# 0kam/alproj

Hardware: AMD Instinct MI355X
Metric: Gpoints/s projected (pinhole + Brown-Conrady, single pose) over the 100M-vertex DSM; CMA-ES iterations/s in `cma` (higher is better)
Workload: dtype f32

## Files before the change

### alproj_amd/csrc/alp_internal.h

```cpp
#pragma once

#include <hip/hip_runtime.h>

#include "host/alp_host.h"
#include "host/alp_buffer.h"

namespace alp {

#define ALP_HIP(expr)                                                                     \
    do {                                                                                  \
        hipError_t e__ = (expr);                                                          \
        if (e__ != hipSuccess)                                                            \
            return ::alp::fail(ALP_EHIP, "%s failed: %s (%s:%d)", #expr,                  \
                               hipGetErrorString(e__), __FILE__, __LINE__);               \
    } while (0)

struct DeviceMemory {
    static int alloc(void **p, size_t bytes) {
        const hipError_t e = hipMalloc(p, bytes);
        return e == hipSuccess ? ALP_OK : fail(ALP_EHIP, "hipMalloc of %zu bytes failed: %s", bytes, hipGetErrorString(e));
    }
    static void release(void *p) { hipFree(p); }
};
struct PinnedMemory {
    static int alloc(void **p, size_t bytes) {
        const hipError_t e = hipHostMalloc(p, bytes, hipHostMallocDefault);
        return e == hipSuccess ? ALP_OK : fail(ALP_EHIP, "hipHostMalloc of %zu bytes failed: %s", bytes, hipGetErrorString(e));
    }
    static void release(void *p) { hipHostFree(p); }
};
template <typename T = void> using DeviceBuffer = Buffer<DeviceMemory, T>;
template <typename T = void> using PinnedBuffer = Buffer<PinnedMemory, T>;

struct Event {
    Event() = default;
    Event(Event &&o) noexcept : e(o.e) { o.e = nullptr; }
    Event &operator=(Event &&o) noexcept {
        std::swap(e, o.e);
        return *this;
    }
    ~Event() {
        if (e) hipEventDestroy(e);
    }
    int ensure() {
        if (!e && hipEventCreate(&e) != hipSuccess) return fail(ALP_EHIP, "hipEventCreate failed");
        return ALP_OK;
    }
    operator hipEvent_t() const { return e; }
    hipEvent_t e = nullptr;
};

struct Context {
    bool ready = false;
    int device = -1;
    int cu_count = 0;
    hipStream_t stream = nullptr;
    hipEvent_t events[64] = {};
    void *scratch = nullptr;
    size_t scratch_cap = 0;
    void *comm = nullptr;
    int rank = 0;
    int world = 1;
};
Context &ctx();
int require_init();
int scratch_reserve(size_t bytes, void **out);

void ktime_begin();
void ktime_end();
struct KTimeScope {
    KTimeScope() { ktime_begin(); }
    ~KTimeScope() { ktime_end(); }
};


const char *raster_dev_flags();

void points_release_staging();

int comm_allreduce_sum_f64(double *dev_buf, int64_t count);

}
```

### alproj_amd/csrc/alp_points.hip

```cpp
#include "alp_internal.h"

#include <algorithm>
#include <cmath>
#include <cstdlib>
#include <vector>

#include "alp_point_kernels.h"
#include "alp_points_internal.h"


using namespace alp;

using alp::host::CONFIRM_MAX;

namespace {

int alloc_planes(DeviceBuffer<> &slab, int k, int64_t n_pad, size_t es, void **planes[]) {
    if (int rc = slab.reserve((size_t)k * n_pad * es)) return rc;
    ALP_HIP(hipMemsetAsync(slab, 0, (size_t)k * n_pad * es, ctx().stream));
    for (int i = 0; i < k; ++i) *planes[i] = (char *)slab + (size_t)i * n_pad * es;
    return ALP_OK;
}

template <typename TIn, typename T>
__global__ __launch_bounds__(256) void column_to_plane_kernel(const TIn *__restrict__ src, int64_t count, int64_t dst_off, double o,
                                                              T *__restrict__ plane) {
    const int64_t stride = (int64_t)gridDim.x * blockDim.x;
    for (int64_t i = (int64_t)blockIdx.x * blockDim.x + threadIdx.x; i < count; i += stride)
        plane[dst_off + i] = (T)((double)src[i] - o);
}

template <typename TIn, typename Launch>
int staged_upload(const void *const *srcs, int nsrc, int64_t n, int width, int64_t CH, Launch launch) {
    const int64_t ch = n < CH ? (n > 0 ? n : 1) : CH;
    DeviceBuffer<TIn> stage;
    if (int rc = stage.reserve((size_t)ch * width * sizeof(TIn))) return rc;
    int rc = ALP_OK;
    for (int c = 0; c < nsrc && !rc; ++c)
        for (int64_t off = 0; off < n; off += ch) {
            const int64_t cnt = (n - off < ch) ? (n - off) : ch;
            hipError_t e = hipMemcpyAsync(stage, (const TIn *)srcs[c] + off * width, (size_t)cnt * width * sizeof(TIn),
                                          hipMemcpyHostToDevice, ctx().stream);
            if (e != hipSuccess) { rc = fail(ALP_EHIP, "H2D upload: %s", hipGetErrorString(e)); break; }
            launch(c, stage, cnt, off, (int)((cnt + 255) / 256 < 4096 ? (cnt + 255) / 256 : 4096));
            e = hipGetLastError();
            if (e != hipSuccess) { rc = fail(ALP_EHIP, "upload kernel: %s", hipGetErrorString(e)); break; }
        }
    if (hipStreamSynchronize(ctx().stream) != hipSuccess && !rc) rc = fail(ALP_EHIP, "upload: stream failed");
    return rc;
}

template <typename TIn, typename T, int C>
int upload_t(const void *rows, const void *const *cols, int64_t n, const double *o, void *const *planes) {
    if (cols)
        return staged_upload<TIn>(cols, C, n, 1, (int64_t)48 << 20, [&](int c, const TIn *stage, int64_t cnt, int64_t off, int grid) {
            hipLaunchKernelGGL((column_to_plane_kernel<TIn, T>), dim3(grid), dim3(256), 0, ctx().stream, stage, cnt, off, o[c], (T *)planes[c]);
        });
    return staged_upload<TIn>(&rows, 1, n, C, (int64_t)16 << 20, [&](int, const TIn *stage, int64_t cnt, int64_t off, int grid) {
        hipLaunchKernelGGL((aos_to_planes_kernel<TIn, T, C>), dim3(grid), dim3(256), 0, ctx().stream, stage, cnt, off, o[0], o[1], o[2],
                           (T *)planes[0], (T *)planes[1], (T *)planes[2]);
    });
}

template <int C>
int upload(const void *rows, const void *const *cols, int in_dtype, int64_t n, const double *o, int precision, void *const *planes) {
    if (in_dtype == ALP_F64 && precision == ALP_F64) return upload_t<double, double, C>(rows, cols, n, o, planes);
    if (in_dtype == ALP_F64 && precision == ALP_F32) return upload_t<double, float, C>(rows, cols, n, o, planes);
    if (in_dtype == ALP_F32 && precision == ALP_F64) return upload_t<float, double, C>(rows, cols, n, o, planes);
    if (in_dtype == ALP_F32 && precision == ALP_F32) return upload_t<float, float, C>(rows, cols, n, o, planes);
    return fail(ALP_EINVAL, "in_dtype must be ALP_F32 or ALP_F64");
}

int stream_grid(int64_t items) { return host::stream_grid(items, ctx().cu_count); }

constexpr uint32_t GRID_MAX_ROW = 64 << 10;
constexpr uint32_t GRID_NONE = 0xffffffffu;

template <typename B>
__global__ __launch_bounds__(256) void grid_row_length_kernel(const B *__restrict__ y, uint32_t n, uint32_t *flags) {
    const B y0 = y[0];
    uint32_t first = GRID_NONE;
    const uint32_t stride = gridDim.x * blockDim.x;
    for (uint32_t i = blockIdx.x * blockDim.x + threadIdx.x; i < n; i += stride)
        if (y[i] != y0) {
            first = i;
            break;
        }
    for (int m = 32; m >= 1; m >>= 1) {
        const uint32_t o = (uint32_t)__shfl_xor((int)first, m);
        first = o < first ? o : first;
    }
    if ((threadIdx.x & 63) == 0 && first != GRID_NONE) atomicMin(flags, first);
}

template <typename B>
__global__ __launch_bounds__(256) void grid_verify_kernel(const B *__restrict__ x, const B *__restrict__ y, uint32_t n, RowDiv rd,
                                                          uint32_t *flags) {
    bool ok = true;
    const uint32_t stride = gridDim.x * blockDim.x;
    for (uint32_t i = blockIdx.x * blockDim.x + threadIdx.x; i < n; i += stride) {
        const uint32_t r = rd.div(i);
        ok &= (x[i] == x[i - r * rd.w]) & (y[i] == y[r * rd.w]);
    }
    if (!ok) atomicOr(flags + 1, 1u);
}

// ... 363 lines not shown
    return comm_allreduce_sum_f64(sums, (int64_t)K * (T + 1));
}

template <typename TS>
int normal_batch_impl(alp_points *p, const std::vector<JacPlan> &plans, int loss, double f_scale, double *out, const int32_t *row_of_pose) {
    const int64_t B = (int64_t)plans.size();
    const int D = plans[0].D, T = D * (D + 1) / 2 + D + 1;
    const host::NormalGrid g = host::normal_batch_grid(p->n, B, ctx().cu_count);
    const size_t plans_bytes = round_up((int64_t)(B * sizeof(JacPlan)), 256), rows_bytes = row_of_pose ? round_up(B * 4, 256) : 0;
    char *dev = nullptr;
    if (int rc = scratch_reserve(plans_bytes + rows_bytes + ((size_t)B * g.blocks * T + (size_t)B * (T + 1)) * sizeof(double), (void **)&dev)) return rc;
    JacPlan *plans_dev = (JacPlan *)dev;
    int *rows_dev = (int *)(dev + plans_bytes);
    double *partials = (double *)(dev + plans_bytes + rows_bytes), *sums = partials + (size_t)B * g.blocks * T;
    hipStream_t st = ctx().stream;
    NormalPosesLaunch l;
    l.timed = true;
    if (g.blocks > 0) {
        const char *order = getenv("ALP_NORMAL_BATCH_ORDER");
        if (order) l.pose_in_x = !strcmp(order, "pose");
        ALP_HIP(hipMemcpyAsync(plans_dev, plans.data(), (size_t)B * sizeof(JacPlan), hipMemcpyHostToDevice, st));
        if (row_of_pose) {
            ALP_HIP(hipMemcpyAsync(rows_dev, row_of_pose, (size_t)B * 4, hipMemcpyHostToDevice, st));
            l.table = true;
            l.row_of_pose = rows_dev;
        }
    }
    if (int rc = normal_poses_enqueue<TS>(p, plans_dev, (int)B, D, g, loss, f_scale, l, partials, sums)) return rc;
    ALP_HIP(hipMemcpyAsync(out, sums, (size_t)B * (T + 1) * sizeof(double), hipMemcpyDeviceToHost, st));
    ALP_HIP(hipStreamSynchronize(st));
    return ALP_OK;
}

}

namespace alp {
int normal_listed_launch(alp_points *p, const JacPlan *plans, const int *list, const long long *count, const int *running, int K, int D,
                         const host::NormalGrid &g, int loss, double f_scale, double *partials, double *sums, bool weight_rows) {
    NormalPosesLaunch l;
    l.list = list, l.count = count, l.running = running, l.pose_in_x = 1, l.table = weight_rows;
    return p->precision == ALP_F64 ? normal_poses_enqueue<double>(p, plans, K, D, g, loss, f_scale, l, partials, sums)
                                   : normal_poses_enqueue<float>(p, plans, K, D, g, loss, f_scale, l, partials, sums);
}
int popeval_launch(alp_points *p, int64_t P, int loss_kind, double f_scale, bool lens_free, bool shared_pose, bool batched,
                   const double *params_dev) {
    return p->precision == ALP_F64 ? popeval_launch_t<double>(p, P, loss_kind, f_scale, lens_free, shared_pose, batched, params_dev)
                                   : popeval_launch_t<float>(p, P, loss_kind, f_scale, lens_free, shared_pose, batched, params_dev);
}
int points_pop_reserve(alp_points *p, int64_t P) { return ensure_pop_scratch(p, P, 0); }
}

namespace {
constexpr int64_t FETCH_CHUNK = (int64_t)8 << 20;
void *g_fetch_stage[2] = {nullptr, nullptr};
hipEvent_t g_fetch_ev[2] = {nullptr, nullptr};

using alp::host::convert_threads;
using alp::host::fetch_threads;

template <typename S, typename D>
__global__ __launch_bounds__(256) void cast_plane_kernel(const S *__restrict__ src, D *__restrict__ dst, long long n) {
    const long long stride = (long long)gridDim.x * blockDim.x;
    for (long long i = (long long)blockIdx.x * blockDim.x + threadIdx.x; i < n; i += stride) dst[i] = (D)src[i];
}

template <typename S, typename D>
int fetch_converted_t(alp_points *p, D *u_out, D *v_out) {
    hipStream_t st = ctx().stream;
    const S *planes[2] = {(const S *)p->u, (const S *)p->v};
    D *outs[2] = {u_out, v_out};
    const char *mode = getenv("ALP_FETCH_CONVERT");
    const bool on_device = mode ? !strcmp(mode, "device") : sizeof(D) < sizeof(S);
    if (on_device) {
        D *tmp = nullptr;
        if (int rc = scratch_reserve((size_t)FETCH_CHUNK * sizeof(D), (void **)&tmp)) return rc;
        for (int pl = 0; pl < 2; ++pl)
            for (int64_t off = 0; off < p->n; off += FETCH_CHUNK) {
                const int64_t cnt = std::min(FETCH_CHUNK, p->n - off);
                hipLaunchKernelGGL((cast_plane_kernel<S, D>), dim3(stream_grid(cnt)), dim3(256), 0, st, planes[pl] + off, tmp, (long long)cnt);
                ALP_HIP(hipMemcpyAsync(outs[pl] + off, tmp, (size_t)cnt * sizeof(D), hipMemcpyDeviceToHost, st));
            }
        ALP_HIP(hipStreamSynchronize(st));
        return ALP_OK;
    }
    for (auto &b : g_fetch_stage)
        if (!b) ALP_HIP(hipHostMalloc(&b, (size_t)FETCH_CHUNK * 8, hipHostMallocDefault));
    const int T = fetch_threads();
    for (auto &e : g_fetch_ev)
        if (!e) ALP_HIP(hipEventCreateWithFlags(&e, hipEventDisableTiming));
    hipEvent_t *ev = g_fetch_ev;
    struct Job { int pl; int64_t off, cnt; };
    std::vector<Job> jobs;
    for (int pl = 0; pl < 2; ++pl)
        for (int64_t off = 0; off < p->n; off += FETCH_CHUNK) jobs.push_back({pl, off, std::min(FETCH_CHUNK, p->n - off)});
    for (size_t k = 0; k <= jobs.size(); ++k) {
        if (k < jobs.size()) {
            const Job &j = jobs[k];
            ALP_HIP(hipMemcpyAsync(g_fetch_stage[k & 1], planes[j.pl] + j.off, (size_t)j.cnt * sizeof(S), hipMemcpyDeviceToHost, st));
            ALP_HIP(hipEventRecord(ev[k & 1], st));
        }
        if (k > 0) {
            const Job &j = jobs[k - 1];
            ALP_HIP(hipEventSynchronize(ev[(k - 1) & 1]));
            convert_threads((const S *)g_fetch_stage[(k - 1) & 1], outs[j.pl] + j.off, j.cnt, T);
        }
    }
    return ALP_OK;
}

}
namespace alp {
void points_release_staging() {
    for (auto &b : g_fetch_stage) {
        if (b) hipHostFree(b);
        b = nullptr;
    }
    for (auto &e : g_fetch_ev) {
        if (e) hipEventDestroy(e);
        e = nullptr;
    }
}
}
namespace {
int fetch_converted(alp_points *p, void *u_out, void *v_out, int out_dtype) {
    return out_dtype == ALP_F64 ? fetch_converted_t<float, double>(p, (double *)u_out, (double *)v_out)
                                : fetch_converted_t<double, float>(p, (float *)u_out, (float *)v_out);
}
}

namespace {
template <typename TIn, typename T>
int weights_stored(const void *w, int64_t n, std::vector<T> &out, double *sum) {
    const TIn *src = (const TIn *)w;
    out.resize((size_t)n);
    double s = 0;
    for (int64_t i = 0; i < n; ++i) {
        const double v = (double)src[i];
        if (!(v >= 0.0) || !std::isfinite(v))
            return fail(ALP_EINVAL, "alp_points_set_weights: weight %lld is negative, NaN or infinite", (long long)i);
        const T t = (T)v;
        if (!std::isfinite((double)t)) return fail(ALP_EINVAL, "alp_points_set_weights: weight %lld does not fit the set's element type", (long long)i);
        out[(size_t)i] = t;
        s += (double)t;
    }
    *sum = s;
    return ALP_OK;
}

template <typename T>
int set_weights_t(alp_points *p, const void *w, int in_dtype) {
    std::vector<T> stored;
    double sum = 0;
    if (int rc = in_dtype == ALP_F64 ? weights_stored<double, T>(w, p->n, stored, &sum) : weights_stored<float, T>(w, p->n, stored, &sum)) return rc;
    if (!p->w) {
        DeviceBuffer<> plane;
        if (int rc = plane.reserve((size_t)p->n_pad * sizeof(T))) return rc;
        hipError_t e = hipMemsetAsync(plane, 0, (size_t)p->n_pad * sizeof(T), ctx().stream);
// ... 503 lines not shown
```

### alproj_amd/csrc/alp_raster.hip

```cpp
#include "alp_raster_internal.h"

#include <algorithm>
#include <atomic>
#include <climits>
#include <cmath>
#include <cstdlib>
#include <thread>
#include <type_traits>
#include <vector>

namespace alp {

#include "raster_dev.h"
#include "raster_common.h"
#include "raster_parked.h"
#include "raster_index.h"
#include "raster_plan.h"
#include "raster_grid.h"
#include "raster_large.h"
#include "raster_resolve.h"
#include "raster_post.h"

}

using namespace alp;

namespace alp {

int upload_chunked(void *dst, const void *src, size_t bytes) {
    const size_t CH = (size_t)256 << 20;
    for (size_t off = 0; off < bytes; off += CH) {
        const size_t n = bytes - off < CH ? bytes - off : CH;
        ALP_HIP(hipMemcpyAsync((char *)dst + off, (const char *)src + off, n, hipMemcpyHostToDevice, ctx().stream));
    }
    ALP_HIP(hipStreamSynchronize(ctx().stream));
    return ALP_OK;
}

template <typename Launch>
static hipError_t staged_upload(const void *src, size_t esize, int64_t total, int64_t chunk, void *stage, Launch launch) {
    for (int64_t off = 0; off < total; off += chunk) {
        const int64_t cnt = total - off < chunk ? total - off : chunk;
        hipError_t e = hipMemcpyAsync(stage, (const char *)src + (size_t)off * esize, (size_t)cnt * esize, hipMemcpyHostToDevice, ctx().stream);
        if (e != hipSuccess) return e;
        launch(off, cnt);
        if ((e = hipGetLastError()) != hipSuccess) return e;
    }
    return hipSuccess;
}

int ensure_queue(alp_mesh *m, unsigned cap) {
    if (m->queue && m->qcap >= cap) return ALP_OK;
    m->qcap = 0;
    if (int rc = m->queue.reserve((size_t)cap * sizeof(WorkItem))) return rc;
    m->qcap = cap;
    return ALP_OK;
}

unsigned initial_queue_cap() { return host::initial_queue_cap(getenv("ALP_QUEUE_CAP")); }
// ... 281 lines not shown
        ALP_HIP(hipMemsetAsync(m->vis, 0, (size_t)v.w * v.h * sizeof(unsigned long long) + QC_TOTAL * sizeof(unsigned), st));
    if (m->n_tri > 0 && !resolve_only) {
        if (m->implicit)
            if (int e = ensure_grid_plan(m, p)) return e;
        if (int e = m->implicit ? draw_grid_mesh(m, v, p) : draw_indexed_mesh(m, v, p)) return e;
    }
    if (int e = m->implicit ? resolve_frame<true>(m, v, rc, min_distance, p) : resolve_frame<false>(m, v, rc, min_distance, p)) return e;
    m->last_v = v;
    m->last_rc = rc;
    m->last_min_distance = min_distance;
    m->unchecked = m->n_tri > 0;
    m->vis_current = true;
    m->rz_n = -1;
    ++(resolve_only ? m->frames_resolve_only : m->frames_full);
    if (int e = dev_report_frame(st)) return e;
    m->rendered = true;
    return ALP_OK;
}

static bool same_view(const View &a, const View &b) {
    return a.w == b.w && a.h == b.h && a.fx == b.fx && a.fy == b.fy && a.sx == b.sx && a.sy == b.sy && a.fxd == b.fxd && a.fyd == b.fyd &&
           !memcmp(a.R, b.R, sizeof(a.R)) && !memcmp(a.camf, b.camf, sizeof(a.camf)) && !memcmp(a.caml, b.caml, sizeof(a.caml)) &&
           !memcmp(a.Rd, b.Rd, sizeof(a.Rd)) && !memcmp(a.camd, b.camd, sizeof(a.camd));
}

int finish_frame(alp_mesh *m) {
    while (m->unchecked) {
        ALP_HIP(hipStreamSynchronize(ctx().stream));
        m->unchecked = false;
        host::FrameQueues have;
        have.items = m->qcap;
        have.general = m->gcap;
        for (int k = 0; k < 3; ++k) {
            have.park[k] = m->park_cap[k];
            have.park_b[k] = m->park_cap_b[k];
        }
        const host::QueueVerdict want = host::frame_verdict(m->qcount_host, QC_STRIDE, m->park_small != nullptr, have);
        if (want.none()) break;
        if (want.park)
            if (int e = alloc_park(m, want.caps.park, want.caps.park_b)) return e;
        if (want.items)
            if (int e = ensure_queue(m, want.caps.items)) return e;
        if (want.general)
            if (int e = ensure_gqueue(m, want.caps.general)) return e;
        if (int e = render_impl(m, m->last_v, m->last_rc, m->last_min_distance)) return e;
    }
    return ALP_OK;
}

}

int alp::finish_frame_of(alp_mesh *m) { return finish_frame(m); }

int alp::upload_f32(float *dst, const void *src, int dtype, int64_t n_vert) {
    const size_t count = (size_t)n_vert * 3;
    if (dtype == ALP_F32) return upload_chunked(dst, src, count * 4);
    const size_t CH = (size_t)24 << 20;
    const size_t ch = count < CH ? count : CH;
    double *stage = nullptr;
    if (int rc = scratch_reserve(ch * 8, (void **)&stage)) return rc;
    hipStream_t st = ctx().stream;
    const hipError_t e = staged_upload(src, 8, (int64_t)count, (int64_t)ch, stage, [&](int64_t off, int64_t cnt) {
        hipLaunchKernelGGL(cast_f64_f32_kernel, dim3(4096), dim3(256), 0, st, stage, (long long)cnt, (long long)off, dst);
    });
    if (e != hipSuccess) return fail(ALP_EHIP, "float64 upload: %s", hipGetErrorString(e));
    ALP_HIP(hipStreamSynchronize(st));
    return ALP_OK;
}

static int streamed_grid_check(alp_mesh *m, const void *ind, int ind_dtype, int64_t n_tri, long long gw, bool *is_grid) {
    hipStream_t st = ctx().stream;
    const size_t esize = ind_dtype == ALP_I32 ? 4 : 8;
    const int64_t total = n_tri * 3;
    const int64_t CH = (int64_t)(((size_t)192 << 20) / esize) / 3 * 3;
    const int64_t ch = total < CH ? total : CH;
    void *stage = nullptr;
    if (int rc = scratch_reserve((size_t)ch * esize, &stage)) return rc;
    hipError_t e = hipMemsetAsync(m->qcount_dev, 0, sizeof(unsigned), st);
    if (e == hipSuccess)
        e = staged_upload(ind, esize, total, ch, stage, [&](int64_t off, int64_t cnt) {
            if (ind_dtype == ALP_I32)
                hipLaunchKernelGGL(check_grid_chunk_kernel<int>, dim3(4096), dim3(256), 0, st, (const int *)stage, cnt / 3, off / 3, gw, m->qcount_dev);
            else
                hipLaunchKernelGGL(check_grid_chunk_kernel<long long>, dim3(4096), dim3(256), 0, st, (const long long *)stage, cnt / 3, off / 3, gw,
                                   m->qcount_dev);
        });
    if (e == hipSuccess) e = hipMemcpyAsync(m->qcount_host, m->qcount_dev, sizeof(unsigned), hipMemcpyDeviceToHost, st);
    if (e == hipSuccess) e = hipStreamSynchronize(st);
    if (e != hipSuccess) return fail(ALP_EHIP, "grid check: %s", hipGetErrorString(e));
    *is_grid = *m->qcount_host == 0;
    return ALP_OK;
}

static int upload_indices(alp_mesh *m, const void *ind, int ind_dtype) {
    hipStream_t st = ctx().stream;
    const long long n_vert = m->n_vert;
    if (int rc = m->ind.reserve((size_t)m->n_tri * 12)) return rc;
    if (hipMemsetAsync(m->qcount_dev, 0, sizeof(unsigned), st) != hipSuccess) return fail(ALP_EHIP, "index check: memset");
    const int64_t total = m->n_tri * 3;
    hipError_t e = hipSuccess;
    if (ind_dtype == ALP_I32) {
        if (int rc = upload_chunked(m->ind, ind, (size_t)total * 4)) return rc;
        hipLaunchKernelGGL(check_index_range_kernel, dim3(4096), dim3(256), 0, st, m->ind, (long long)total, n_vert, m->qcount_dev);
    } else {
        const int64_t CH = 24 << 20;
        const int64_t ch = total < CH ? total : CH;
        long long *stage = nullptr;
        if (int rc = scratch_reserve((size_t)ch * 8, (void **)&stage)) return rc;
        e = staged_upload(ind, 8, total, ch, stage, [&](int64_t off, int64_t cnt) {
            hipLaunchKernelGGL(narrow_indices_kernel, dim3(4096), dim3(256), 0, st, stage, (long long)cnt, (long long)off, m->ind, n_vert,
                               m->qcount_dev);
        });
    }
    if (e == hipSuccess) e = hipGetLastError();
    if (e == hipSuccess) e = hipMemcpyAsync(m->qcount_host, m->qcount_dev, sizeof(unsigned), hipMemcpyDeviceToHost, st);
    if (e == hipSuccess) e = hipStreamSynchronize(st);
    if (e != hipSuccess) return fail(ALP_EHIP, "index upload: %s", hipGetErrorString(e));
    if (*m->qcount_host == 0) return ALP_OK;
    for (int64_t i = 0; i < total; ++i) {
        const long long v = ind_dtype == ALP_I32 ? (long long)((const int *)ind)[i] : ((const long long *)ind)[i];
        if (v < 0 || v >= n_vert) return fail(ALP_EINVAL, "index %lld out of range at %lld", v, (long long)i);
    }
    return fail(ALP_EINVAL, "%u indices out of range", *m->qcount_host);
}

using alp::host::HostGridCheck;
using alp::host::host_check_threads;

extern "C" {

int alp_mesh_create(const void *vert, int vert_dtype, const void *value, int value_dtype, int64_t n_vert, const void *ind,
                    int ind_dtype, int64_t n_tri, int64_t grid_h, int64_t grid_w, alp_mesh_t **out) {
    if (int rc = require_init()) return rc;
    ALP_REQUIRE(out, "out is NULL");
    *out = nullptr;
    ALP_REQUIRE(vert && n_vert > 0, "vert is NULL or empty");
    ALP_REQUIRE(vert_dtype == ALP_F32 || vert_dtype == ALP_F64, "vert_dtype must be ALP_F32 or ALP_F64");
    ALP_REQUIRE(!value || value_dtype == ALP_F32 || value_dtype == ALP_F64, "value_dtype must be ALP_F32 or ALP_F64");
    ALP_REQUIRE(n_vert < ((int64_t)1 << 31), "more than 2^31 vertices");
    const bool implicit = ind == nullptr;
    if (implicit) {
        ALP_REQUIRE(grid_h >= 2 && grid_w >= 2 && grid_h * grid_w == n_vert, "implicit grid: grid_h*grid_w != n_vert");
        n_tri = 2 * (grid_h - 1) * (grid_w - 1);
    } else {
        ALP_REQUIRE(ind_dtype == ALP_I32 || ind_dtype == ALP_I64, "ind_dtype must be ALP_I32 or ALP_I64");
        ALP_REQUIRE(n_tri >= 0, "n_tri is negative");
    }
    ALP_REQUIRE(n_tri < ((int64_t)1 << 32) - 1, "more than 2^32-2 triangles");
    alp_mesh *m = new alp_mesh();
    m->n_vert = n_vert;
    m->n_tri = n_tri;
    m->grid_h = grid_h;
// ... 385 lines not shown
```

### alproj_amd/csrc/host/alp_host.h

```cpp
#pragma once

#include <algorithm>
#include <atomic>
#include <cmath>
#include <cstdarg>
#include <cstdint>
#include <cstdio>
#include <cstdlib>
#include <cstring>
#include <thread>
#include <vector>

#include "alproj_hip.h"

#if defined(__SANITIZE_THREAD__)
#define ALP_TSAN_BUILD 1
#elif defined(__has_feature)
#if __has_feature(thread_sanitizer)
#define ALP_TSAN_BUILD 1
#endif
#endif
#ifndef ALP_TSAN_BUILD
#define ALP_TSAN_BUILD 0
#endif
// ... 42 lines not shown
int fold_pose_jacobian(const double params[ALP_NPARAM], const double origin[3], const int32_t *target, int D, double *jac);

struct alignas(16) JacPlan {
    double rec[POSE_WORDS];
    double drow[JAC_MAX][12];
    double lens_f[JAC_MAX];
    double su, sv;
    int32_t lens_w[JAC_MAX];
    int32_t D;
};
int jacobian_plan(const double params[ALP_NPARAM], const double origin[3], const int32_t *target, int D, int of_residuals,
                  JacPlan *plan);

}
#include "host/alp_jacplan.h"
#include "host/alp_lm.h"
namespace alp {

namespace host {

constexpr int64_t HASH_SLICE_BYTES = (int64_t)8 << 20;
constexpr int64_t MINMAX_VALUES_PER_THREAD = (int64_t)1 << 20;
uint64_t hash64(const void *buf, int64_t bytes, int threads);
void minmax(const double *values, int64_t n, int threads, double out[2]);
void prefault(void *buf, int64_t bytes, int threads);

template <typename S, typename D>
inline void convert_slice(const S *__restrict__ src, D *__restrict__ dst, int64_t n) {
#if defined(__has_builtin) && __has_builtin(__builtin_nontemporal_store) && !ALP_TSAN_BUILD
    for (int64_t i = 0; i < n; ++i) __builtin_nontemporal_store((D)src[i], dst + i);
#else
    for (int64_t i = 0; i < n; ++i) dst[i] = (D)src[i];
#endif
}

constexpr int64_t CONVERT_SERIAL_BELOW = 1 << 16;

template <typename S, typename D>
inline void convert_threads(const S *src, D *dst, int64_t n, int T) {
    if (T <= 1 || n < CONVERT_SERIAL_BELOW) return convert_slice(src, dst, n);
    std::vector<std::thread> th;
    const int64_t per = ((n + T - 1) / T + 15) & ~(int64_t)15;
    for (int t = 1; t < T; ++t) {
        const int64_t a = std::min(n, per * t), b = std::min(n, per * (t + 1));
        if (b > a) th.emplace_back([=] { convert_slice(src + a, dst + a, b - a); });
    }
    convert_slice(src, dst, std::min(n, per));
    for (auto &x : th) x.join();
}

inline int fetch_threads() {
    if (const char *e = getenv("ALP_HOST_THREADS")) return std::max(1, std::min(64, atoi(e)));
    return (int)std::max(1u, std::min(16u, std::thread::hardware_concurrency()));
}

template <typename I>
inline void grid_rows_check(const I *ind, long long gw, long long row0, long long row1, std::atomic<bool> *bad) {
    const long long gc = gw - 1;
    for (long long r = row0; r < row1 && !bad->load(std::memory_order_relaxed); ++r) {
        const I *p = ind + (size_t)r * gc * 6;
        long long a = r * gw;
        bool diff = false;
        for (long long c = 0; c < gc; ++c, ++a, p += 6)
            diff |= (long long)p[0] != a || (long long)p[1] != a + gw || (long long)p[2] != a + gw + 1 || (long long)p[3] != a ||
                    (long long)p[4] != a + gw + 1 || (long long)p[5] != a + 1;
        if (diff) bad->store(true, std::memory_order_relaxed);
    }
}

struct HostGridCheck {
    std::vector<std::thread> threads;
    std::atomic<bool> bad{false};
    bool started = false;
    void start(const void *ind, int ind_dtype, long long gh, long long gw, int n_threads) {
        const long long rows = gh - 1;
        const int T = (int)std::min<long long>(n_threads, rows);
        try {
            for (int t = 0; t < T; ++t) {
                const long long r0 = rows * t / T, r1 = rows * (t + 1) / T;
                if (ind_dtype == ALP_I32) threads.emplace_back(grid_rows_check<int>, (const int *)ind, gw, r0, r1, &bad);
                else threads.emplace_back(grid_rows_check<long long>, (const long long *)ind, gw, r0, r1, &bad);
            }
            started = true;
        } catch (...) {
            bad.store(true);
            join();
            bad.store(false);
            started = false;
        }
    }
    void join() {
        for (auto &t : threads)
            if (t.joinable()) t.join();
        threads.clear();
    }
    bool is_grid() {
        join();
        return started && !bad.load();
    }
    ~HostGridCheck() { bad.store(true); join(); }
};

inline int host_check_threads(int64_t n_tri) {
    if (const char *e = getenv("ALP_HOST_THREADS")) return std::max(0, std::min(64, atoi(e)));
    if (n_tri < (1 << 18)) return 0;
    const unsigned hc = std::thread::hardware_concurrency();
// ... 73 lines not shown
```

### alproj_amd/csrc/host/alp_host_selfcheck.cpp

```cpp
#include <cinttypes>
#include <mutex>
#include <random>
#include <string>
#include <utility>

#include "host/alp_host.h"
#include "host/alp_buffer.h"

using namespace alp;

namespace {

std::atomic<int> g_failures{0};
std::mutex g_print;

#define CHECK(cond, ...)                                           \
    do {                                                           \
        if (!(cond)) {                                             \
            std::lock_guard<std::mutex> lk(g_print);               \
            fprintf(stderr, "CHECK FAILED %s:%d: %s | ", __FILE__, __LINE__, #cond); \
            fprintf(stderr, __VA_ARGS__);                          \
            fprintf(stderr, "\n");                                 \
            g_failures.fetch_add(1);                               \
        }                                                          \
// ... 111 lines not shown
        for (int k = 0; k < 8; ++k) {
            const double q[3] = {2000 * U(rng), 2000 * U(rng), 300 * U(rng)};
            const double P[3] = {origin[0] + q[0] - p[0], origin[1] + q[1] - p[1], origin[2] + q[2] - p[2]};
            double cam[3];
            for (int i = 0; i < 3; ++i) cam[i] = R[i][0] * P[0] + R[i][1] * P[1] + R[i][2] * P[2];
            const double x = fx * cam[0] + p[23] * cam[2], y = fy * cam[1] + p[24] * cam[2], z = cam[2];
            const double x1 = ((w - x / z) - c0) / c0, y1 = (y / z - c1) / c1;
            const double zf = rec[8] * q[0] + rec[9] * q[1] + rec[10] * q[2] + rec[11];
            const double x1f = (rec[0] * q[0] + rec[1] * q[1] + rec[2] * q[2] + rec[3]) / zf;
            const double y1f = (rec[4] * q[0] + rec[5] * q[1] + rec[6] * q[2] + rec[7]) / zf;
            if (std::fabs(z) < 1) continue;
            CHECK(std::fabs(x1f - x1) <= 1e-9 * std::max(1.0, std::fabs(x1)), "x1 %.17g vs %.17g", x1f, x1);
            CHECK(std::fabs(y1f - y1) <= 1e-9 * std::max(1.0, std::fabs(y1)), "y1 %.17g vs %.17g", y1f, y1);
            double pl[ALP_NPARAM];
            memcpy(pl, p, sizeof(pl));
            for (int i = 9; i <= 20; ++i) pl[i] = 0;
            CHECK(pose_is_lens_free(pl) && !pose_is_lens_free(p), "pose_is_lens_free");
            double lf[POSE_WORDS];
            fold_pose_lens_free(pl, origin, lf);
            const double uo = 5616 * U(rng), vo = 3744 * U(rng);
            const double u_ref = c0 * x1 + c0, v_ref = c1 * (y1 * (1 + pl[7]) / (1 + pl[8])) + c1;
            const double zl = lf[8] * q[0] + lf[9] * q[1] + lf[10] * q[2] + lf[11];
            const double du = (uo - lf[26]) + (lf[0] * q[0] + lf[1] * q[1] + lf[2] * q[2] + lf[3]) / zl;
            const double dv = (vo - lf[27]) + (lf[4] * q[0] + lf[5] * q[1] + lf[6] * q[2] + lf[7]) / zl;
            CHECK(std::fabs(du - (uo - u_ref)) <= 1e-8 * std::max(1.0, std::fabs(u_ref)), "lens-free du %.17g vs %.17g", du, uo - u_ref);
            CHECK(std::fabs(dv - (vo - v_ref)) <= 1e-8 * std::max(1.0, std::fabs(v_ref)), "lens-free dv %.17g vs %.17g", dv, vo - v_ref);
            CHECK(zl == zf && lf[26] == c0 && lf[27] == c1 && lf[12] == 0 && lf[31] == 0, "lens-free record layout");
        }
    }
}

template <typename S, typename D>
void check_convert_t() {
    const int64_t lim = host::CONVERT_SERIAL_BELOW;
    const int64_t sizes[] = {0, 1, 15, 16, 17, lim - 1, lim, lim + 1, 70001, (1 << 20) + 3};
    std::mt19937_64 rng(4);
    std::uniform_real_distribution<double> U(-1e7, 1e7);
    for (int64_t n : sizes) {
        std::vector<S> src((size_t)n);
        for (auto &x : src) x = (S)U(rng);
        for (int T : THREAD_COUNTS) {
            std::vector<D> dst((size_t)n, (D)-1);
            host::convert_threads(src.data(), dst.data(), n, T);
            bool same = true;
            for (int64_t i = 0; i < n; ++i) same &= dst[(size_t)i] == (D)src[(size_t)i];
            CHECK(same, "convert n=%" PRId64 " T=%d", n, T);
        }
    }
}

void check_convert() {
    check_convert_t<float, double>();
    check_convert_t<double, float>();
}

template <typename I>
std::vector<I> grid_indices(long long gh, long long gw) {
    std::vector<I> ind;
    ind.reserve((size_t)((gh - 1) * (gw - 1) * 6));
    for (long long r = 0; r + 1 < gh; ++r)
        for (long long c = 0; c + 1 < gw; ++c) {
            const long long a = r * gw + c;
            for (long long v : {a, a + gw, a + gw + 1, a, a + gw + 1, a + 1}) ind.push_back((I)v);
        }
    return ind;
}

template <typename I>
void check_grid_t(int dtype) {
    const long long shapes[][2] = {{2, 2}, {3, 5}, {17, 4}, {2, 300}, {300, 251}};
    for (auto &sh : shapes) {
        const long long gh = sh[0], gw = sh[1];
        std::vector<I> ind = grid_indices<I>(gh, gw);
        const int64_t n_tri = (int64_t)ind.size() / 3, n_vert = gh * gw;
        long long cgh = 0, cgw = 0;
        CHECK(host::grid_candidate(ind.data(), dtype, n_tri, n_vert, &cgh, &cgw) && cgh == gh && cgw == gw, "candidate %lld x %lld", gh, gw);
        CHECK(!host::grid_candidate(ind.data(), dtype, n_tri - 1, n_vert, &cgh, &cgw), "odd triangle count accepted");
        CHECK(!host::grid_candidate(ind.data(), dtype, n_tri, n_vert + 1, &cgh, &cgw) || (n_vert + 1) % gw == 0, "wrong vertex count accepted");
        for (int T : {1, 2, 8, 64}) {
            {
                host::HostGridCheck chk;
                chk.start(ind.data(), dtype, gh, gw, T);
                CHECK(chk.is_grid(), "grid %lld x %lld not recognised (T=%d)", gh, gw, T);
            }
            for (size_t at : {(size_t)0, ind.size() / 2, ind.size() - 1}) {
                const I keep = ind[at];
                ind[at] = (I)(keep + 1);
                {
                    host::HostGridCheck chk;
                    chk.start(ind.data(), dtype, gh, gw, T);
                    CHECK(!chk.is_grid(), "wrong entry %zu of a %lld x %lld grid not seen (T=%d)", at, gh, gw, T);
                }
                ind[at] = keep;
            }
            {
                host::HostGridCheck chk;
                chk.start(ind.data(), dtype, gh, gw, T);
            }
            {
                host::HostGridCheck chk;
                CHECK(!chk.is_grid(), "a check that never ran says grid");
            }
        }
    }
}

// ... 657 lines not shown
    }
    {
        Bytes a;
        CHECK(a.reserve(16) == ALP_OK, "reserve");
        unsigned char *pa = a;
        Bytes b(std::move(a));
        CHECK(!a && a.capacity() == 0 && b.get() == pa && b.capacity() == 16 && Mem::live == 1, "move construction");
        Bytes c;
        c = std::move(b);
        CHECK(!b && c.get() == pa && c.capacity() == 16 && Mem::live == 1, "move assignment to an empty buffer");
        Bytes d;
        CHECK(d.reserve(32) == ALP_OK && Mem::live == 2, "reserve");
        d = std::move(c);
        CHECK(!c && d.get() == pa && d.capacity() == 16 && Mem::live == 1, "move assignment onto a block left %d live", Mem::live);
        Bytes &self = d;
        d = std::move(self);
        CHECK(d.get() == pa && Mem::live == 1, "self-assignment");
        Buffer<Mem> v;
        CHECK(v.reserve(8) == ALP_OK && (const float *)v == (const float *)v.get() && (char *)v + 4 == (char *)v.get() + 4, "casts");
    }
    CHECK(Mem::live == 0, "%d block(s) outlived their buffers", Mem::live);
    for (int size = 2; size <= 3; ++size)
        for (int bad = 1; bad <= size; ++bad)
            for (int held = 0; held < 2; ++held) {
                Buffer<Mem, double> x;
                Buffer<Mem> y;
                Buffer<Mem, int> z;
                auto group = [&](size_t n) {
                    return size == 2 ? reserve_all({n, 2 * n}, x, y) : reserve_all({n, 2 * n, 3 * n}, x, y, z);
                };
                if (held) CHECK(group(8) == ALP_OK && Mem::live == size, "first group");
                Mem::fail_next(bad);
                CHECK(group(64) == ALP_EHIP && !x && !y && !z && x.capacity() + y.capacity() + z.capacity() == 0 && Mem::live == 0,
                      "group of %d, member %d failed (held %d): %d block(s) live", size, bad, held, Mem::live);
                Mem::fail_next(0);
                CHECK(group(64) == ALP_OK && x && y && (size == 2 || z) && x.capacity() == 64 && y.capacity() == 128,
                      "group of %d after a failure", size);
                CHECK(Mem::live == size, "group of %d after a failure: %d blocks", size, Mem::live);
                x[7] = 1.0;
                ((char *)y)[127] = 1;
                if (size == 3) z[47] = 1;
                double *px = x;
                CHECK(group(64) == ALP_OK && x.get() == px && Mem::live == size, "a group that fits moved");
                reset_all(x, y, z);
                CHECK(Mem::live == 0, "reset_all");
            }
    CHECK(Mem::live == 0, "%d block(s) live at the end", Mem::live);
}

int main(int argc, char **argv) {
    if (argc > 2 && !strcmp(argv[1], "--canary")) return canary(argv[2]);
    if (argc > 1 && !strcmp(argv[1], "--plan")) return plan(argc - 2, argv + 2);
    if (argc > 1 && !strcmp(argv[1], "--lm")) return lm_mode();
    struct Group { const char *name; void (*fn)(); };
    const Group groups[] = {{"hash", check_hash},     {"minmax", check_minmax},   {"prefault", check_prefault}, {"fold_pose", check_fold_pose},
                            {"convert", check_convert}, {"grid", check_grid},     {"selection", check_selection}, {"errors", check_errors},
                            {"plan", check_plan},       {"frame_plan", check_frame_plan}, {"row_div", check_row_div}, {"lm", check_lm},
                            {"buffer", check_buffer},   {"row_walk", check_row_walk}, {"match_plan", check_match_plan}};
    const bool concurrent = !(argc > 1 && !strcmp(argv[1], "--serial"));
    std::vector<std::thread> th;
    for (const Group &g : groups) {
        if (concurrent) th.emplace_back(g.fn);
        else g.fn();
    }
    for (auto &x : th) x.join();
    std::thread a(check_convert), b(check_convert);
    check_selection();
    a.join();
    b.join();
    if (g_failures.load()) {
        fprintf(stderr, "host selfcheck: %d comparison(s) failed\n", g_failures.load());
        return 1;
    }
    printf("host selfcheck ok: %zu groups%s\n", sizeof(groups) / sizeof(groups[0]), concurrent ? ", run concurrently" : "");
    return 0;
}
```

Baseline: 502.1.

## Narrow float64 coordinates and int64 indices on host before upload

Adds a host-side multithreaded narrowing path that converts float64 vertex columns (optionally subtracting an origin) and int64 triangle indices to 32-bit values in pinned double-buffered staging. The narrowed data is copied to the device with async copies that overlap the next chunk's conversion. This halves the bytes crossing PCIe and drops the device-side conversion kernels. In exchange it uses host CPU threads and moves the index range check to the host. The staging buffers are now shared with the fetch path.

After: 499.8. Within noise of the previous version (-0.5%).

```diff
diff --git a/alproj_amd/csrc/alp_internal.h b/alproj_amd/csrc/alp_internal.h
--- a/alproj_amd/csrc/alp_internal.h
+++ b/alproj_amd/csrc/alp_internal.h
@@ -76,7 +76,43 @@
 
 const char *raster_dev_flags();
 
+constexpr size_t HOST_STAGE_BYTES = (size_t)64 << 20;
+int host_staging(void *stage[2], hipEvent_t ev[2]);
 void points_release_staging();
+
+inline bool narrow_on_host() {
+    const char *mode = getenv("ALP_UPLOAD_CONVERT");
+    return !mode || strcmp(mode, "device") != 0;
+}
+
+inline int64_t narrow_chunk_values() {
+    const int64_t most = (int64_t)(HOST_STAGE_BYTES / 4);
+    const char *e = getenv("ALP_UPLOAD_CHUNK");
+    return e ? std::max<int64_t>(1, std::min<int64_t>(most, atoll(e))) : most;
+}
+
+template <typename Narrow>
+inline int upload_narrowed(void *dst, int64_t total, Narrow narrow) {
+    void *stage[2];
+    hipEvent_t ev[2];
+    if (int rc = host_staging(stage, ev)) return rc;
+    hipStream_t st = ctx().stream;
+    const int64_t ch = narrow_chunk_values();
+    hipError_t e = hipSuccess;
+    int64_t k = 0;
+    for (int64_t off = 0; off < total && e == hipSuccess; off += ch, ++k) {
+        const int64_t cnt = std::min(ch, total - off);
+        const int b = (int)(k & 1);
+        if (k >= 2) e = hipEventSynchronize(ev[b]);
+        if (e != hipSuccess || !narrow(off, cnt, stage[b])) break;
+        e = hipMemcpyAsync((char *)dst + (size_t)off * 4, stage[b], (size_t)cnt * 4, hipMemcpyHostToDevice, st);
+        if (e == hipSuccess) e = hipEventRecord(ev[b], st);
+    }
+    const hipError_t e_sync = hipStreamSynchronize(st);
+    if (e == hipSuccess) e = e_sync;
+    if (e != hipSuccess) return fail(ALP_EHIP, "narrowing upload: %s", hipGetErrorString(e));
+    return ALP_OK;
+}
 
 int comm_allreduce_sum_f64(double *dev_buf, int64_t count);
 
diff --git a/alproj_amd/csrc/alp_points.hip b/alproj_amd/csrc/alp_points.hip
--- a/alproj_amd/csrc/alp_points.hip
+++ b/alproj_amd/csrc/alp_points.hip
@@ -3,6 +3,7 @@
 #include <algorithm>
 #include <cmath>
 #include <cstdlib>
+#include <type_traits>
 #include <vector>
 
 #include "alp_point_kernels.h"
@@ -52,6 +53,20 @@
 
 template <typename TIn, typename T, int C>
 int upload_t(const void *rows, const void *const *cols, int64_t n, const double *o, void *const *planes) {
+    if constexpr (std::is_same<TIn, double>::value && std::is_same<T, float>::value)
+        if (cols && narrow_on_host()) {
+            const int threads = host::upload_threads();
+            for (int c = 0; c < C; ++c) {
+                const double *col = (const double *)cols[c];
+                const double oc = o[c];
+                if (int rc = upload_narrowed(planes[c], n, [=](int64_t off, int64_t cnt, void *stage) {
+                        host::narrow_sub_f32_threads(col + off, oc, (float *)stage, cnt, threads);
+                        return true;
+                    }))
+                    return rc;
+            }
+            return ALP_OK;
+        }
     if (cols)
         return staged_upload<TIn>(cols, C, n, 1, (int64_t)48 << 20, [&](int c, const TIn *stage, int64_t cnt, int64_t off, int grid) {
             hipLaunchKernelGGL((column_to_plane_kernel<TIn, T>), dim3(grid), dim3(256), 0, ctx().stream, stage, cnt, off, o[c], (T *)planes[c]);
@@ -521,11 +536,25 @@
 
 namespace {
 constexpr int64_t FETCH_CHUNK = (int64_t)8 << 20;
+static_assert(FETCH_CHUNK * 8 == alp::HOST_STAGE_BYTES, "a chunk of float64 fills a staging buffer");
 void *g_fetch_stage[2] = {nullptr, nullptr};
 hipEvent_t g_fetch_ev[2] = {nullptr, nullptr};
 
 using alp::host::convert_threads;
 using alp::host::fetch_threads;
+
+}
+namespace alp {
+int host_staging(void *stage[2], hipEvent_t ev[2]) {
+    for (auto &b : g_fetch_stage)
+        if (!b) ALP_HIP(hipHostMalloc(&b, (size_t)HOST_STAGE_BYTES, hipHostMallocDefault));
+    for (auto &e : g_fetch_ev)
+        if (!e) ALP_HIP(hipEventCreateWithFlags(&e, hipEventDisableTiming));
+    for (int b = 0; b < 2; ++b) stage[b] = g_fetch_stage[b], ev[b] = g_fetch_ev[b];
+    return ALP_OK;
+}
+}
+namespace {
 
 template <typename S, typename D>
 __global__ __launch_bounds__(256) void cast_plane_kernel(const S *__restrict__ src, D *__restrict__ dst, long long n) {
@@ -552,12 +581,10 @@
         ALP_HIP(hipStreamSynchronize(st));
         return ALP_OK;
     }
-    for (auto &b : g_fetch_stage)
-        if (!b) ALP_HIP(hipHostMalloc(&b, (size_t)FETCH_CHUNK * 8, hipHostMallocDefault));
+    hipEvent_t ev[2];
+    void *stage[2];
+    if (int rc = host_staging(stage, ev)) return rc;
     const int T = fetch_threads();
-    for (auto &e : g_fetch_ev)
-        if (!e) ALP_HIP(hipEventCreateWithFlags(&e, hipEventDisableTiming));
-    hipEvent_t *ev = g_fetch_ev;
     struct Job { int pl; int64_t off, cnt; };
     std::vector<Job> jobs;
     for (int pl = 0; pl < 2; ++pl)
@@ -565,13 +592,13 @@
     for (size_t k = 0; k <= jobs.size(); ++k) {
         if (k < jobs.size()) {
             const Job &j = jobs[k];
-            ALP_HIP(hipMemcpyAsync(g_fetch_stage[k & 1], planes[j.pl] + j.off, (size_t)j.cnt * sizeof(S), hipMemcpyDeviceToHost, st));
+            ALP_HIP(hipMemcpyAsync(stage[k & 1], planes[j.pl] + j.off, (size_t)j.cnt * sizeof(S), hipMemcpyDeviceToHost, st));
             ALP_HIP(hipEventRecord(ev[k & 1], st));
         }
         if (k > 0) {
             const Job &j = jobs[k - 1];
             ALP_HIP(hipEventSynchronize(ev[(k - 1) & 1]));
-            convert_threads((const S *)g_fetch_stage[(k - 1) & 1], outs[j.pl] + j.off, j.cnt, T);
+            convert_threads((const S *)stage[(k - 1) & 1], outs[j.pl] + j.off, j.cnt, T);
         }
     }
     return ALP_OK;
diff --git a/alproj_amd/csrc/alp_raster.hip b/alproj_amd/csrc/alp_raster.hip
--- a/alproj_amd/csrc/alp_raster.hip
+++ b/alproj_amd/csrc/alp_raster.hip
@@ -5,6 +5,7 @@
 #include <climits>
 #include <cmath>
 #include <cstdlib>
+#include <cstring>
 #include <thread>
 #include <type_traits>
 #include <vector>
@@ -392,9 +393,17 @@
 
 int alp::finish_frame_of(alp_mesh *m) { return finish_frame(m); }
 
+
 int alp::upload_f32(float *dst, const void *src, int dtype, int64_t n_vert) {
     const size_t count = (size_t)n_vert * 3;
     if (dtype == ALP_F32) return upload_chunked(dst, src, count * 4);
+    if (narrow_on_host()) {
+        const int T = host::upload_threads();
+        return upload_narrowed(dst, (int64_t)count, [=](int64_t off, int64_t cnt, void *stage) {
+            host::narrow_f32_threads((const double *)src + off, (float *)stage, cnt, T);
+            return true;
+        });
+    }
     const size_t CH = (size_t)24 << 20;
     const size_t ch = count < CH ? count : CH;
     double *stage = nullptr;
@@ -436,8 +445,19 @@
     hipStream_t st = ctx().stream;
     const long long n_vert = m->n_vert;
     if (int rc = m->ind.reserve((size_t)m->n_tri * 12)) return rc;
+    const int64_t total = m->n_tri * 3;
+    if (ind_dtype == ALP_I64 && narrow_on_host()) {
+        const int T = host::upload_threads();
+        host::IndexNarrow found;
+        if (int rc = upload_narrowed(m->ind, total, [&](int64_t off, int64_t cnt, void *stage) {
+                host::narrow_indices_threads((const long long *)ind + off, (int32_t *)stage, cnt, off, n_vert, T, &found);
+                return found.bad == 0;
+            }))
+            return rc;
+        if (found.bad) return fail(ALP_EINVAL, "index %lld out of range at %lld", found.first_value, found.first_at);
+        return ALP_OK;
+    }
     if (hipMemsetAsync(m->qcount_dev, 0, sizeof(unsigned), st) != hipSuccess) return fail(ALP_EHIP, "index check: memset");
-    const int64_t total = m->n_tri * 3;
     hipError_t e = hipSuccess;
     if (ind_dtype == ALP_I32) {
         if (int rc = upload_chunked(m->ind, ind, (size_t)total * 4)) return rc;
diff --git a/alproj_amd/csrc/host/alp_host.h b/alproj_amd/csrc/host/alp_host.h
--- a/alproj_amd/csrc/host/alp_host.h
+++ b/alproj_amd/csrc/host/alp_host.h
@@ -118,6 +118,94 @@
 inline int fetch_threads() {
     if (const char *e = getenv("ALP_HOST_THREADS")) return std::max(1, std::min(64, atoi(e)));
     return (int)std::max(1u, std::min(16u, std::thread::hardware_concurrency()));
+}
+
+
+inline int upload_threads() { return std::min(16, fetch_threads()); }
+
+template <typename F>
+inline int for_each_share(int64_t n, int T, F fn) {
+    if (T <= 1 || n < CONVERT_SERIAL_BELOW) {
+        fn(0, (int64_t)0, n);
+        return 1;
+    }
+    const int64_t per = ((n + T - 1) / T + 15) & ~(int64_t)15;
+    std::vector<std::thread> th;
+    for (int t = 1; t < T; ++t) {
+        const int64_t a = std::min(n, per * t), b = std::min(n, per * (t + 1));
+        if (b > a) th.emplace_back([=] { fn(t, a, b); });
+    }
+    fn(0, (int64_t)0, std::min(n, per));
+    for (auto &x : th) x.join();
+    return T;
+}
+
+template <bool SUB>
+inline void narrow_f32_slice_t(const double *__restrict__ src, double o, float *__restrict__ dst, int64_t n) {
+    auto one = [o](double v) { return SUB ? (float)(v - o) : (float)v; };
+    int64_t i = 0;
+#if defined(__clang__) && defined(__has_builtin) && __has_builtin(__builtin_nontemporal_store) && __has_builtin(__builtin_convertvector) && !ALP_TSAN_BUILD
+    typedef double d4 __attribute__((ext_vector_type(4)));
+    typedef float f4 __attribute__((ext_vector_type(4)));
+    for (; i < n && ((uintptr_t)(dst + i) & 15); ++i) dst[i] = one(src[i]);
+    for (; i + 4 <= n; i += 4) {
+        d4 v;
+        memcpy(&v, src + i, sizeof(v));
+        if (SUB) v = v - o;
+        __builtin_nontemporal_store(__builtin_convertvector(v, f4), (f4 *)(dst + i));
+    }
+#endif
+    for (; i < n; ++i) dst[i] = one(src[i]);
+}
+
+inline void narrow_f32_threads(const double *src, float *dst, int64_t n, int T) {
+    for_each_share(n, T, [=](int, int64_t a, int64_t b) { narrow_f32_slice_t<false>(src + a, 0.0, dst + a, b - a); });
+}
+
+inline void narrow_sub_f32_threads(const double *src, double o, float *dst, int64_t n, int T) {
+    for_each_share(n, T, [=](int, int64_t a, int64_t b) { narrow_f32_slice_t<true>(src + a, o, dst + a, b - a); });
+}
+
+struct IndexNarrow {
+    long long bad = 0;
+    long long first_at = -1, first_value = 0;
+};
+
+inline long long narrow_indices_slice(const long long *__restrict__ src, int32_t *__restrict__ dst, int64_t n, long long n_vert,
+                                      int64_t *first) {
+    long long bad = 0;
+    int64_t at = INT64_MAX;
+    for (int64_t i = 0; i < n; ++i) {
+        const long long v = src[i];
+        const bool out = (unsigned long long)v >= (unsigned long long)n_vert;
+        bad += out;
+        at = std::min(at, out ? i : INT64_MAX);
+        const int32_t low = (int32_t)(uint32_t)(unsigned long long)v;
+#if defined(__has_builtin) && __has_builtin(__builtin_nontemporal_store) && !ALP_TSAN_BUILD
+        __builtin_nontemporal_store(low, dst + i);
+#else
+        dst[i] = low;
+#endif
+    }
+    *first = at;
+    return bad;
+}
+
+inline void narrow_indices_threads(const long long *src, int32_t *dst, int64_t n, int64_t base, long long n_vert, int T, IndexNarrow *acc) {
+    struct Found { long long bad = 0; int64_t at = INT64_MAX; };
+    std::vector<Found> found((size_t)std::max(1, T));
+    Found *f = found.data();
+    for_each_share(n, T, [=](int t, int64_t a, int64_t b) {
+        f[t].bad = narrow_indices_slice(src + a, dst + a, b - a, n_vert, &f[t].at);
+        if (f[t].at != INT64_MAX) f[t].at += a;
+    });
+    for (const Found &x : found) {
+        if (x.bad && acc->first_at < 0) {
+            acc->first_at = base + x.at;
+            acc->first_value = src[x.at];
+        }
+        acc->bad += x.bad;
+    }
 }
 
 template <typename I>
diff --git a/alproj_amd/csrc/host/alp_host_selfcheck.cpp b/alproj_amd/csrc/host/alp_host_selfcheck.cpp
--- a/alproj_amd/csrc/host/alp_host_selfcheck.cpp
+++ b/alproj_amd/csrc/host/alp_host_selfcheck.cpp
@@ -187,6 +187,175 @@
 void check_convert() {
     check_convert_t<float, double>();
     check_convert_t<double, float>();
+}
+
+std::vector<std::pair<int64_t, int>> narrow_cases() {
+    const int64_t lim = host::CONVERT_SERIAL_BELOW;
+    std::vector<std::pair<int64_t, int>> cases;
+    for (int64_t n : {(int64_t)0, (int64_t)1, (int64_t)15, (int64_t)16, (int64_t)17, lim - 1, lim, lim + 1, (int64_t)70001})
+        for (int T : {1, 2, 3, 7, 16}) cases.push_back({n, T});
+    for (int T = 1; T <= 16; ++T) {
+        const int64_t whole = 16 * T * ((lim + 16 * T - 1) / (16 * T));
+        for (int64_t n : {whole - T, whole - 1, whole, whole + 1}) cases.push_back({n, T});
+    }
+    return cases;
+}
+
+void check_narrow_f32() {
+    const uint64_t bits[] = {0x0000000000000000ull, 0x8000000000000000ull,
+                             0x36A0000000000000ull, 0x369FFFFFFFFFFFFFull,
+                             0x380FFFFFC0000000ull, 0x3810000000000000ull,
+                             0x47EFFFFFE0000000ull, 0x47EFFFFFF0000000ull,
+                             0x4810000000000000ull, 0xC810000000000000ull,
+                             0x7FF8000000000000ull, 0xFFF0000000000000ull,
+                             0x3FF0000010000000ull, 0x3FF0000030000000ull,
+                             0x3FF0000010000001ull, 0x3FD5555555555555ull};
+    const int n_bits = (int)(sizeof(bits) / sizeof(bits[0]));
+    std::mt19937_64 rng(11);
+    std::uniform_real_distribution<double> U(-1e7, 1e7);
+    for (const auto &c : narrow_cases()) {
+        const int64_t n = c.first;
+        const int T = c.second;
+        std::vector<double> src((size_t)n);
+        for (int64_t i = 0; i < n; ++i) {
+            src[(size_t)i] = U(rng);
+            if (i % 5 == 0) memcpy(&src[(size_t)i], &bits[(i / 5) % n_bits], 8);
+        }
+        if (n > 0) memcpy(&src[(size_t)n - 1], &bits[7], 8);
+        {
+            std::vector<float> dst((size_t)n, -1.0f);
+            host::narrow_f32_threads(src.data() + 0, dst.data(), n, T);
+            bool same = true;
+            for (int64_t i = 0; i < n; ++i) {
+                const float want = (float)src[(size_t)i];
+                same &= !memcmp(&dst[(size_t)i], &want, 4);
+            }
+            CHECK(same, "narrow f32 n=%" PRId64 " T=%d", n, T);
+        }
+    }
+    for (const auto &c : narrow_cases()) {
+        const int64_t n = c.first;
+        const int T = c.second;
+        if (n == 0 || (n > 17 && T != 1 && T != 5 && T != 16)) continue;
+        for (double o : {732000.123, -4048018.5, 0.0, 1e39}) {
+            std::vector<double> src((size_t)n);
+            for (int64_t i = 0; i < n; ++i) {
+                src[(size_t)i] = o + U(rng) * 1e-3;
+                if (i % 7 == 0) memcpy(&src[(size_t)i], &bits[(i / 7) % n_bits], 8);
+            }
+            src[(size_t)n - 1] = o + 1 + ldexp(1.0, -24);
+            std::vector<float> dst((size_t)n, -1.0f);
+            host::narrow_sub_f32_threads(src.data(), o, dst.data(), n, T);
+            bool same = true;
+            for (int64_t i = 0; i < n; ++i) {
+                const volatile double diff = src[(size_t)i] - o;
+                const float want = (float)diff;
+                same &= !memcmp(&dst[(size_t)i], &want, 4);
+            }
+            CHECK(same, "narrow f32 with origin %g n=%" PRId64 " T=%d", o, n, T);
+        }
+    }
+    const struct { uint64_t in; uint32_t out; } want[] = {
+        {bits[0], 0x00000000u}, {bits[1], 0x80000000u}, {bits[2], 0x00000001u}, {bits[3], 0x00000001u}, {0x3690000000000000ull, 0x00000000u},
+        {bits[4], 0x007FFFFFu}, {bits[5], 0x00800000u}, {bits[6], 0x7F7FFFFFu}, {bits[7], 0x7F800000u}, {bits[8], 0x7F800000u},
+        {bits[9], 0xFF800000u}, {bits[11], 0xFF800000u}, {bits[12], 0x3F800000u}, {bits[13], 0x3F800002u}, {bits[14], 0x3F800001u}};
+    for (const auto &w : want) {
+        double d;
+        float f = -1.0f;
+        uint32_t got;
+        memcpy(&d, &w.in, 8);
+        host::narrow_f32_threads(&d, &f, 1, 4);
+        memcpy(&got, &f, 4);
+        CHECK(got == w.out, "float64 %016" PRIx64 " -> %08x, expected %08x", w.in, got, w.out);
+    }
+    double nan_in;
+    float nan_out = 0;
+    memcpy(&nan_in, &bits[10], 8);
+    host::narrow_f32_threads(&nan_in, &nan_out, 1, 1);
+    CHECK(nan_out != nan_out, "NaN stays NaN");
+    CHECK(host::upload_threads() >= 1 && host::upload_threads() <= 16, "upload_threads() = %d", host::upload_threads());
+}
+
+void check_narrow_indices() {
+    const long long n_vert = 1000003;
+    const long long offenders[] = {-1, n_vert, (1ll << 31), (1ll << 32) + 5, (1ll << 32), -(1ll << 32) + 7, (1ll << 62) + 1, INT64_MIN, INT64_MAX};
+    std::mt19937_64 rng(12);
+    for (const auto &c : narrow_cases()) {
+        const int64_t n = c.first;
+        const int T = c.second;
+        std::vector<long long> src((size_t)n);
+        for (auto &x : src) x = (long long)(rng() % (uint64_t)n_vert);
+        if (n > 2) src[0] = 0, src[(size_t)n - 1] = n_vert - 1;
+        {
+            const int64_t per = ((n + T - 1) / T + 15) & ~(int64_t)15;
+            std::vector<std::vector<int64_t>> plants = {{}};
+            if (n > 0) plants.push_back({n - 1}), plants.push_back({0});
+            if (n > 3) plants.push_back({n - 1, n / 2}), plants.push_back({1, n - 2, n / 3});
+            if (n >= host::CONVERT_SERIAL_BELOW && T > 1)
+                for (int64_t t = 1; t < T && per * t < n; t += (T > 4 ? 3 : 1)) plants.push_back({per * t}), plants.push_back({per * t - 1, per * t});
+            int which = T;
+            for (const auto &at : plants) {
+                std::vector<long long> a = src;
+                for (int64_t p : at) a[(size_t)p] = offenders[(size_t)(which++) % (sizeof(offenders) / sizeof(offenders[0]))];
+                std::vector<int32_t> dst((size_t)n, -7);
+                host::IndexNarrow found;
+                const int64_t base = 3 * n + 1;
+                host::narrow_indices_threads(a.data(), dst.data(), n, base, n_vert, T, &found);
+                long long bad = 0, first = -1;
+                bool same = true;
+                for (int64_t i = 0; i < n; ++i) {
+                    const long long v = a[(size_t)i];
+                    if (v < 0 || v >= n_vert) {
+                        ++bad;
+                        if (first < 0) first = i;
+                    } else {
+                        same &= (long long)dst[(size_t)i] == v;
+                    }
+                }
+                CHECK(same, "narrow indices n=%" PRId64 " T=%d: a valid index changed", n, T);
+                CHECK(found.bad == bad, "narrow indices n=%" PRId64 " T=%d: %lld counted, %lld planted", n, T, found.bad, bad);
+                CHECK(found.first_at == (first < 0 ? -1 : base + first) && (first < 0 || found.first_value == a[(size_t)first]),
+                      "narrow indices n=%" PRId64 " T=%d: first offender at %lld (%lld), expected %lld", n, T, found.first_at, found.first_value,
+                      first < 0 ? -1 : base + first);
+                if (bad && n > 0) {
+                    host::narrow_indices_threads(a.data(), dst.data(), n, base + n, n_vert, T, &found);
+                    CHECK(found.bad == 2 * bad && found.first_at == base + first, "narrow indices n=%" PRId64 " T=%d: second chunk", n, T);
+                }
+            }
+        }
+    }
+}
+
+int narrow_mode(int argc, char **argv) {
+    if (argc == 1 && !strcmp(argv[0], "threads")) {
+        printf("%d\n", host::upload_threads());
+        return 0;
+    }
+    if (argc < 4) return 2;
+    const bool f32 = !strcmp(argv[0], "f32");
+    FILE *in = fopen(argv[1], "rb");
+    if (!in) return 2;
+    fseek(in, 0, SEEK_END);
+    const int64_t n = (int64_t)ftell(in) / 8;
+    fseek(in, 0, SEEK_SET);
+    std::vector<uint64_t> src((size_t)n + 1);
+    if (n && fread(src.data() + 1, 8, (size_t)n, in) != (size_t)n) return 2;
+    fclose(in);
+    std::vector<uint32_t> dst((size_t)n);
+    const int T = atoi(argv[3]);
+    if (f32 && argc > 4) {
+        host::narrow_sub_f32_threads((const double *)(src.data() + 1), strtod(argv[4], nullptr), (float *)dst.data(), n, T);
+    } else if (f32) {
+        host::narrow_f32_threads((const double *)(src.data() + 1), (float *)dst.data(), n, T);
+    } else {
+        host::IndexNarrow found;
+        host::narrow_indices_threads((const long long *)(src.data() + 1), (int32_t *)dst.data(), n, 0, argc > 4 ? atoll(argv[4]) : 1, T, &found);
+        printf("%lld %lld %lld\n", found.bad, found.first_at, found.first_value);
+    }
+    FILE *out = fopen(argv[2], "wb");
+    if (!out || (n && fwrite(dst.data(), 4, (size_t)n, out) != (size_t)n)) return 2;
+    fclose(out);
+    return 0;
 }
 
 template <typename I>
@@ -950,11 +1119,13 @@
     if (argc > 2 && !strcmp(argv[1], "--canary")) return canary(argv[2]);
     if (argc > 1 && !strcmp(argv[1], "--plan")) return plan(argc - 2, argv + 2);
     if (argc > 1 && !strcmp(argv[1], "--lm")) return lm_mode();
+    if (argc > 1 && !strcmp(argv[1], "--narrow")) return narrow_mode(argc - 2, argv + 2);
     struct Group { const char *name; void (*fn)(); };
     const Group groups[] = {{"hash", check_hash},     {"minmax", check_minmax},   {"prefault", check_prefault}, {"fold_pose", check_fold_pose},
                             {"convert", check_convert}, {"grid", check_grid},     {"selection", check_selection}, {"errors", check_errors},
                             {"plan", check_plan},       {"frame_plan", check_frame_plan}, {"row_div", check_row_div}, {"lm", check_lm},
-                            {"buffer", check_buffer},   {"row_walk", check_row_walk}, {"match_plan", check_match_plan}};
+                            {"buffer", check_buffer},   {"row_walk", check_row_walk}, {"match_plan", check_match_plan},
+                            {"narrow_f32", check_narrow_f32}, {"narrow_indices", check_narrow_indices}};
     const bool concurrent = !(argc > 1 && !strcmp(argv[1], "--serial"));
     std::vector<std::thread> th;
     for (const Group &g : groups) {
```
